# real-stanford/garmentnets

Measured on AMD Instinct MI355X. Metric: garments/s end-to-end predict (PointNet++ -> gridding -> UNet3D -> WNF decode -> marching cubes), higher is better.
Workload: dtype f32 (f16x2 convs, f16x2 decoder MLPs, fp32 accumulation)

## Files before the change

garmentnets_amd/csrc/upconv.hip:

```cpp
#include "split_conv.h"

struct UpArgs {
    const float *src;
    const float *a, *d;
    const uint4 *wp;
    const float *out_scale;
    const float *act_inv;
    float *partial;
    int C1, B, Dc, Hc, Wc, Cout;
    int tiles_y, tiles_x;
};

template <int NT, bool F16>
__global__ __launch_bounds__(512, 1) void upconv_partial_kernel(UpArgs p) {
    constexpr int TZC = NT == 1 ? 2 : 1, NF = 2 * TZC, HZ = TZC + 2, HVOX = HZ * 100;
    using HL = HaloLayout<2, HZ>;
    constexpr int NIT = (HVOX * 4 + 511) / 512;
    __shared__ __attribute__((aligned(16))) unsigned char smem[2 * HL::BYTES + 2 * 384 * 4];
    float *const adl = reinterpret_cast<float *>(smem + 2 * HL::BYTES);
    const int tid = threadIdx.x, lane = tid & 63, h = lane >> 5, r = lane & 31;
    const int cls = __builtin_amdgcn_readfirstlane(tid >> 6), pz = cls >> 2, py = (cls >> 1) & 1, px = cls & 1;
    const unsigned nblk = gridDim.x, xcd = blockIdx.x & 7u, jx = blockIdx.x >> 3, qx = nblk >> 3, rx = nblk & 7u;
    const unsigned logical = (xcd < rx ? xcd * (qx + 1) : rx * (qx + 1) + (xcd - rx) * qx) + jx;
    const int ncb = p.Cout / (32 * NT);
    int tile = (int)(logical / (unsigned)ncb);
    const int cb = (int)(logical % (unsigned)ncb);
    const int tiles_z = (p.Dc + TZC - 1) / TZC;
    const int tz = tile % tiles_z; tile /= tiles_z;
    const int tx = tile % p.tiles_x; tile /= p.tiles_x;
    const int ty = tile;
    const int z0 = tz * TZC, y0 = ty * 8, x0 = tx * 8;
    const int b = blockIdx.y;
    const int nslices = p.C1 / 16;
    const int nblocks = p.Cout / 32;

    f32x16 acc[NF][NT], tot[NF][NT];
#pragma unroll
    for (int f = 0; f < NF; ++f)
#pragma unroll
        for (int u = 0; u < NT; ++u)
#pragma unroll
            for (int q = 0; q < 16; ++q) { acc[f][u][q] = 0.f; tot[f][u][q] = 0.f; }
    for (int i = tid; i < p.C1; i += 512) { adl[i] = p.a[(int64_t)b * p.C1 + i]; adl[384 + i] = p.d[(int64_t)b * p.C1 + i]; }

    const int c4 = (tid & 3) * 4;
    float4 raw[NIT];
    unsigned inb = 0;
    auto issue_rows = [&](int sl) {
        inb = 0;
#pragma unroll
        for (int it = 0; it < NIT; ++it) {
            const int idx = tid + it * 512;
            const int hv = (idx < HVOX * 4 ? idx : HVOX * 4 - 1) >> 2;
            const int hx = hv % 10, hy = (hv / 10) % 10, hz = hv / 100;
            const int gz = z0 + hz - 1, gy = y0 + hy - 1, gx = x0 + hx - 1;
            const bool in = idx < HVOX * 4 && gz >= 0 && gz < p.Dc && gy >= 0 && gy < p.Hc && gx >= 0 && gx < p.Wc;
            raw[it] = make_float4(0.f, 0.f, 0.f, 0.f);
            if (in) {
                raw[it] = *reinterpret_cast<const float4 *>(p.src + ((((int64_t)b * p.Dc + gz) * p.Hc + gy) * p.Wc + gx) * p.C1 + sl * 16 + c4);
                inb |= 1u << it;
            }
        }
    };
    auto convert_row = [&](int it, int sl, int buf) {
        const int idx = tid + it * 512;
        if (idx < HVOX * 4) {
            const int hv = idx >> 2;
            const float4 av = *reinterpret_cast<const float4 *>(adl + sl * 16 + c4);
            const float4 dv = *reinterpret_cast<const float4 *>(adl + 384 + sl * 16 + c4);
            float v0 = 0.f, v1 = 0.f, v2 = 0.f, v3 = 0.f;
            if (inb & (1u << it)) {
                v0 = __fmaf_rn(raw[it].x, av.x, dv.x);
                v1 = __fmaf_rn(raw[it].y, av.y, dv.y);
                v2 = __fmaf_rn(raw[it].z, av.z, dv.z);
                v3 = __fmaf_rn(raw[it].w, av.w, dv.w);
            }
            uint2 pl[2];
            split4<2, F16>(v0, v1, v2, v3, pl);
            unsigned char *dst = smem + buf * HL::BYTES + HL::at(hv / 100, (hv / 10) % 10, hv % 10) + c4 * 2;
            *reinterpret_cast<uint2 *>(dst) = pl[0];
            *reinterpret_cast<uint2 *>(dst + 32) = pl[1];
        }
    };

    issue_rows(0);
    __syncthreads();
#pragma unroll
    for (int it = 0; it < NIT; ++it) convert_row(it, 0, 0);
    __syncthreads();

    const int64_t bstep = (int64_t)8 * nblocks * 2 * 64;
    const uint4 *bw = p.wp + ((int64_t)cls * nblocks + cb * NT) * 2 * 64 + lane;
    uint4 bf[NT][2], nbf[NT][2], nnbf[NT][2];
#pragma unroll
    for (int u = 0; u < NT; ++u) { nbf[u][0] = bw[(u * 2 + 0) * 64]; nbf[u][1] = bw[(u * 2 + 1) * 64]; }
    bw += bstep;
#pragma unroll
    for (int u = 0; u < NT; ++u) { nnbf[u][0] = bw[(u * 2 + 0) * 64]; nnbf[u][1] = bw[(u * 2 + 1) * 64]; }
    bw += bstep;
    const int abase = HL::at(pz, (r >> 3) + py, (r & 7) + px) + 16 * h;
    constexpr int AF1 = 4 * HL::ROWP, AFZ = 10 * HL::ROWP;
    const int nsteps = nslices * 8;
    int step = 0;
    uint4 af[NF][2], naf[NF][2];
#pragma unroll
    for (int f = 0; f < NF; ++f) {
        naf[f][0] = *reinterpret_cast<const uint4 *>(smem + abase + (f >> 1) * AFZ + (f & 1) * AF1);
        naf[f][1] = *reinterpret_cast<const uint4 *>(smem + abase + (f >> 1) * AFZ + (f & 1) * AF1 + 32);
    }
    for (int s = 0; s < nslices; ++s) {
        const unsigned char *const halo = smem + (s & 1) * HL::BYTES, *const halo_n = smem + ((s + 1) & 1) * HL::BYTES;
        const bool more = s + 1 < nslices;
        if (more) issue_rows(s + 1);
#pragma unroll
        for (int tap = 0; tap < 8; ++tap, ++step) {
#pragma unroll
            for (int u = 0; u < NT; ++u) { bf[u][0] = nbf[u][0]; bf[u][1] = nbf[u][1]; nbf[u][0] = nnbf[u][0]; nbf[u][1] = nnbf[u][1]; }
#pragma unroll
            for (int f = 0; f < NF; ++f) { af[f][0] = naf[f][0]; af[f][1] = naf[f][1]; }
            if (step + 2 < nsteps) {
#pragma unroll
                for (int u = 0; u < NT; ++u) { nnbf[u][0] = bw[(u * 2 + 0) * 64]; nnbf[u][1] = bw[(u * 2 + 1) * 64]; }
                bw += bstep;
            }
            if (tap < 7) {
                const int toff = HL::at((tap + 1) >> 2, ((tap + 1) >> 1) & 1, (tap + 1) & 1);
#pragma unroll
                for (int f = 0; f < NF; ++f) {
                    naf[f][0] = *reinterpret_cast<const uint4 *>(halo + abase + toff + (f >> 1) * AFZ + (f & 1) * AF1);
                    naf[f][1] = *reinterpret_cast<const uint4 *>(halo + abase + toff + (f >> 1) * AFZ + (f & 1) * AF1 + 32);
                }
            }
#define UP_PROD(IA, IB)                                                                                                        \
            _Pragma("unroll") for (int u = 0; u < NT; ++u)                                                                     \
                _Pragma("unroll") for (int f = 0; f < NF; ++f) acc[f][u] = mfma16<F16>(af[f][IA], bf[u][IB], acc[f][u]);
            UP_PROD(1, 0)
            if (more && tap >= 2 && tap < 2 + NIT) convert_row(tap - 2, s + 1, (s + 1) & 1);
            UP_PROD(0, 1) UP_PROD(0, 0)
#undef UP_PROD
        }
#pragma unroll
        for (int f = 0; f < NF; ++f)
#pragma unroll
            for (int u = 0; u < NT; ++u)
#pragma unroll
                for (int q = 0; q < 16; ++q) { tot[f][u][q] = __fadd_rn(tot[f][u][q], acc[f][u][q]); acc[f][u][q] = 0.f; }
        __syncthreads();
        if (more) {
#pragma unroll
            for (int f = 0; f < NF; ++f) {
                naf[f][0] = *reinterpret_cast<const uint4 *>(halo_n + abase + (f >> 1) * AFZ + (f & 1) * AF1);
                naf[f][1] = *reinterpret_cast<const uint4 *>(halo_n + abase + (f >> 1) * AFZ + (f & 1) * AF1 + 32);
            }
        }
    }
    const int64_t pc = (int64_t)8 * p.Cout;
#pragma unroll
    for (int f = 0; f < NF; ++f)
#pragma unroll
        for (int u = 0; u < NT; ++u) {
            const int t = f & 1, gz = z0 + (f >> 1);
            const int n = cls * p.Cout + (cb * NT + u) * 32 + r;
            const float osc = p.act_inv ? __fmul_rn(p.out_scale[n], p.act_inv[b]) : p.out_scale[n];
            if (z0 + TZC <= p.Dc && y0 + 8 <= p.Hc && x0 + 8 <= p.Wc) {
                float *ob = p.partial + ((((int64_t)b * p.Dc + gz) * p.Hc + (y0 + t * 4)) * p.Wc + (x0 + 4 * h)) * pc + n;
                const int64_t rs = (int64_t)p.Wc * pc;
#pragma unroll
                for (int q = 0; q < 16; ++q) ob[(q >> 2) * rs + (q & 3) * pc] = __fmul_rn(tot[f][u][q], osc);
                continue;
            }
#pragma unroll
            for (int q = 0; q < 16; ++q) {
                const int i = (q & 3) + 8 * (q >> 2) + 4 * h;
                const int gy = y0 + t * 4 + (i >> 3), gx = x0 + (i & 7);
                if (gz < p.Dc && gy < p.Hc && gx < p.Wc)
                    p.partial[((((int64_t)b * p.Dc + gz) * p.Hc + gy) * p.Wc + gx) * pc + n] = __fmul_rn(tot[f][u][q], osc);
            }
        }
}

extern "C" int gn_upconv_partial(const float *src1, int C1, const float *a, const float *d, const void *wp, int mode, const float *out_scale,
                                 const float *act_inv_scale, int B, int Dc, int Hc, int Wc, int Cout, float *partial, void *stream) {
    GN_REQUIRE(B >= 0 && Dc > 0 && Hc > 0 && Wc > 0 && C1 > 0 && Cout > 0, "gn_upconv_partial: bad sizes");
    GN_REQUIRE(mode == GN_SPLIT_BF16X2 || mode == GN_SPLIT_F16X2, "gn_upconv_partial: two-plane modes only (GN_SPLIT_BF16X2 / GN_SPLIT_F16X2)");
    GN_REQUIRE(C1 % 16 == 0 && C1 <= 384 && Cout % 32 == 0, "gn_upconv_partial: channels must be multiples of 16 (in, <= 384) / 32 (out)");
    if (B == 0) return GN_OK;
    GN_REQUIRE(src1 && a && d && wp && out_scale && partial, "gn_upconv_partial: null pointer");
    UpArgs p;
    p.src = src1; p.a = a; p.d = d; p.wp = (const uint4 *)wp; p.out_scale = out_scale; p.act_inv = act_inv_scale; p.partial = partial;
    p.C1 = C1; p.B = B; p.Dc = Dc; p.Hc = Hc; p.Wc = Wc; p.Cout = Cout;
    p.tiles_y = (int)gn_cdiv(Hc, 8); p.tiles_x = (int)gn_cdiv(Wc, 8);
    hipStream_t st = gn_stream(stream);
    const bool f16 = mode == GN_SPLIT_F16X2;
    if (Cout % 64 == 0) {
        const unsigned g = (unsigned)(gn_cdiv(Dc, 1) * p.tiles_y * p.tiles_x * (Cout / 64));
        if (f16) hipLaunchKernelGGL((upconv_partial_kernel<2, true>), dim3(g, B), dim3(512), 0, st, p);
        else hipLaunchKernelGGL((upconv_partial_kernel<2, false>), dim3(g, B), dim3(512), 0, st, p);
    } else {
        const unsigned g = (unsigned)(gn_cdiv(Dc, 2) * p.tiles_y * p.tiles_x * (Cout / 32));
        if (f16) hipLaunchKernelGGL((upconv_partial_kernel<1, true>), dim3(g, B), dim3(512), 0, st, p);
        else hipLaunchKernelGGL((upconv_partial_kernel<1, false>), dim3(g, B), dim3(512), 0, st, p);
    }
    GN_LAUNCH_CHECK("gn_upconv_partial");
    return GN_OK;
}
```

Measured before the change: 155.5.

## Make upconv kernel persistent with cross-tile prefetch of halo and weights

Converts the transposed-conv partial kernel into a persistent kernel launched with one block per CU (rounded to a multiple of 8). Each block loops over work items and overlaps the next tile's halo load, weight prefetch and per-sample affine table with the current tile's last slice. This is meant to hide the prologue and epilogue latency between tiles and to remove the cost of per-block launch and ramp-up. In exchange it adds complex control flow, a double-buffered affine table that uses more LDS, and possible load imbalance.

```diff
diff --git a/garmentnets_amd/csrc/upconv.hip b/garmentnets_amd/csrc/upconv.hip
--- a/garmentnets_amd/csrc/upconv.hip
+++ b/garmentnets_amd/csrc/upconv.hip
@@ -9,6 +9,7 @@
     float *partial;
     int C1, B, Dc, Hc, Wc, Cout;
     int tiles_y, tiles_x;
+    unsigned items_per_sample, n_items;
 };
 
 template <int NT, bool F16>
@@ -16,23 +17,27 @@
     constexpr int TZC = NT == 1 ? 2 : 1, NF = 2 * TZC, HZ = TZC + 2, HVOX = HZ * 100;
     using HL = HaloLayout<2, HZ>;
     constexpr int NIT = (HVOX * 4 + 511) / 512;
-    __shared__ __attribute__((aligned(16))) unsigned char smem[2 * HL::BYTES + 2 * 384 * 4];
+    __shared__ __attribute__((aligned(16))) unsigned char smem[2 * HL::BYTES + 2 * 2 * 384 * 4];
     float *const adl = reinterpret_cast<float *>(smem + 2 * HL::BYTES);
     const int tid = threadIdx.x, lane = tid & 63, h = lane >> 5, r = lane & 31;
     const int cls = __builtin_amdgcn_readfirstlane(tid >> 6), pz = cls >> 2, py = (cls >> 1) & 1, px = cls & 1;
-    const unsigned nblk = gridDim.x, xcd = blockIdx.x & 7u, jx = blockIdx.x >> 3, qx = nblk >> 3, rx = nblk & 7u;
-    const unsigned logical = (xcd < rx ? xcd * (qx + 1) : rx * (qx + 1) + (xcd - rx) * qx) + jx;
     const int ncb = p.Cout / (32 * NT);
-    int tile = (int)(logical / (unsigned)ncb);
-    const int cb = (int)(logical % (unsigned)ncb);
     const int tiles_z = (p.Dc + TZC - 1) / TZC;
-    const int tz = tile % tiles_z; tile /= tiles_z;
-    const int tx = tile % p.tiles_x; tile /= p.tiles_x;
-    const int ty = tile;
-    const int z0 = tz * TZC, y0 = ty * 8, x0 = tx * 8;
-    const int b = blockIdx.y;
     const int nslices = p.C1 / 16;
     const int nblocks = p.Cout / 32;
+    auto decode = [&](unsigned v, int &b_, int &cb_, int &z0_, int &y0_, int &x0_) {
+        const unsigned nblk = p.items_per_sample, bq = v / nblk, i = v - bq * nblk;
+        const unsigned xcd = i & 7u, jx = i >> 3, qx = nblk >> 3, rx = nblk & 7u;
+        const unsigned logical = (xcd < rx ? xcd * (qx + 1) : rx * (qx + 1) + (xcd - rx) * qx) + jx;
+        int tile = (int)(logical / (unsigned)ncb);
+        cb_ = (int)(logical % (unsigned)ncb);
+        const int tz = tile % tiles_z; tile /= tiles_z;
+        const int tx = tile % p.tiles_x; tile /= p.tiles_x;
+        b_ = (int)bq; z0_ = tz * TZC; y0_ = tile * 8; x0_ = tx * 8;
+    };
+    unsigned item = blockIdx.x;
+    int b, cb, z0, y0, x0;
+    decode(item, b, cb, z0, y0, x0);
 
     f32x16 acc[NF][NT], tot[NF][NT];
 #pragma unroll
@@ -41,33 +46,35 @@
         for (int u = 0; u < NT; ++u)
 #pragma unroll
             for (int q = 0; q < 16; ++q) { acc[f][u][q] = 0.f; tot[f][u][q] = 0.f; }
-    for (int i = tid; i < p.C1; i += 512) { adl[i] = p.a[(int64_t)b * p.C1 + i]; adl[384 + i] = p.d[(int64_t)b * p.C1 + i]; }
-
-    const int c4 = (tid & 3) * 4;
+
     float4 raw[NIT];
     unsigned inb = 0;
-    auto issue_rows = [&](int sl) {
+    auto issue_rows = [&](int b_, int z0_, int y0_, int x0_, int sl) {
         inb = 0;
+        int tl = threadIdx.x;
+        asm volatile("" : "+v"(tl));
 #pragma unroll
         for (int it = 0; it < NIT; ++it) {
-            const int idx = tid + it * 512;
+            const int idx = tl + it * 512;
             const int hv = (idx < HVOX * 4 ? idx : HVOX * 4 - 1) >> 2;
             const int hx = hv % 10, hy = (hv / 10) % 10, hz = hv / 100;
-            const int gz = z0 + hz - 1, gy = y0 + hy - 1, gx = x0 + hx - 1;
+            const int gz = z0_ + hz - 1, gy = y0_ + hy - 1, gx = x0_ + hx - 1;
             const bool in = idx < HVOX * 4 && gz >= 0 && gz < p.Dc && gy >= 0 && gy < p.Hc && gx >= 0 && gx < p.Wc;
             raw[it] = make_float4(0.f, 0.f, 0.f, 0.f);
             if (in) {
-                raw[it] = *reinterpret_cast<const float4 *>(p.src + ((((int64_t)b * p.Dc + gz) * p.Hc + gy) * p.Wc + gx) * p.C1 + sl * 16 + c4);
+                raw[it] = *reinterpret_cast<const float4 *>(p.src + ((((int64_t)b_ * p.Dc + gz) * p.Hc + gy) * p.Wc + gx) * p.C1 + sl * 16 + (tl & 3) * 4);
                 inb |= 1u << it;
             }
         }
     };
-    auto convert_row = [&](int it, int sl, int buf) {
-        const int idx = tid + it * 512;
+    auto convert_row = [&](int it, int sl, int buf, int tab) {
+        int tl = threadIdx.x;
+        asm volatile("" : "+v"(tl));
+        const int idx = tl + it * 512, c4 = (tl & 3) * 4;
         if (idx < HVOX * 4) {
             const int hv = idx >> 2;
-            const float4 av = *reinterpret_cast<const float4 *>(adl + sl * 16 + c4);
-            const float4 dv = *reinterpret_cast<const float4 *>(adl + 384 + sl * 16 + c4);
+            const float4 av = *reinterpret_cast<const float4 *>(adl + tab * 768 + sl * 16 + c4);
+            const float4 dv = *reinterpret_cast<const float4 *>(adl + tab * 768 + 384 + sl * 16 + c4);
             float v0 = 0.f, v1 = 0.f, v2 = 0.f, v3 = 0.f;
             if (inb & (1u << it)) {
                 v0 = __fmaf_rn(raw[it].x, av.x, dv.x);
@@ -83,100 +90,131 @@
         }
     };
 
-    issue_rows(0);
-    __syncthreads();
-#pragma unroll
-    for (int it = 0; it < NIT; ++it) convert_row(it, 0, 0);
-    __syncthreads();
-
     const int64_t bstep = (int64_t)8 * nblocks * 2 * 64;
-    const uint4 *bw = p.wp + ((int64_t)cls * nblocks + cb * NT) * 2 * 64 + lane;
+    auto bw_first = [&](int cb_) { return p.wp + ((int64_t)cls * nblocks + cb_ * NT) * 2 * 64 + lane; };
+    const uint4 *bw = nullptr;
     uint4 bf[NT][2], nbf[NT][2], nnbf[NT][2];
-#pragma unroll
-    for (int u = 0; u < NT; ++u) { nbf[u][0] = bw[(u * 2 + 0) * 64]; nbf[u][1] = bw[(u * 2 + 1) * 64]; }
-    bw += bstep;
-#pragma unroll
-    for (int u = 0; u < NT; ++u) { nnbf[u][0] = bw[(u * 2 + 0) * 64]; nnbf[u][1] = bw[(u * 2 + 1) * 64]; }
-    bw += bstep;
     const int abase = HL::at(pz, (r >> 3) + py, (r & 7) + px) + 16 * h;
     constexpr int AF1 = 4 * HL::ROWP, AFZ = 10 * HL::ROWP;
-    const int nsteps = nslices * 8;
-    int step = 0;
     uint4 af[NF][2], naf[NF][2];
-#pragma unroll
-    for (int f = 0; f < NF; ++f) {
-        naf[f][0] = *reinterpret_cast<const uint4 *>(smem + abase + (f >> 1) * AFZ + (f & 1) * AF1);
-        naf[f][1] = *reinterpret_cast<const uint4 *>(smem + abase + (f >> 1) * AFZ + (f & 1) * AF1 + 32);
+    const int64_t pc = (int64_t)8 * p.Cout;
+    bool fresh = true;
+    int buf = 0, tab = 0;
+    for (;;) {
+        const unsigned nitem = item + gridDim.x;
+        const bool more = nitem < p.n_items;
+        int bn = b, cbn = cb, z0n = z0, y0n = y0, x0n = x0;
+        if (more) decode(nitem, bn, cbn, z0n, y0n, x0n);
+        const bool cont = more && (bn == b || nslices >= 2);
+        const int tabn = bn == b ? tab : tab ^ 1;
+        if (fresh) {
+            __syncthreads();
+            for (int i = tid; i < p.C1; i += 512) { adl[tab * 768 + i] = p.a[(int64_t)b * p.C1 + i]; adl[tab * 768 + 384 + i] = p.d[(int64_t)b * p.C1 + i]; }
+            issue_rows(b, z0, y0, x0, 0);
+            __syncthreads();
+            buf = 0;
+#pragma unroll
+            for (int it = 0; it < NIT; ++it) convert_row(it, 0, 0, tab);
+            __syncthreads();
+            bw = bw_first(cb);
+#pragma unroll
+            for (int u = 0; u < NT; ++u) { nbf[u][0] = bw[(u * 2 + 0) * 64]; nbf[u][1] = bw[(u * 2 + 1) * 64]; }
+            bw += bstep;
+#pragma unroll
+            for (int u = 0; u < NT; ++u) { nnbf[u][0] = bw[(u * 2 + 0) * 64]; nnbf[u][1] = bw[(u * 2 + 1) * 64]; }
+            bw += bstep;
+#pragma unroll
+            for (int f = 0; f < NF; ++f) {
+                naf[f][0] = *reinterpret_cast<const uint4 *>(smem + abase + (f >> 1) * AFZ + (f & 1) * AF1);
+                naf[f][1] = *reinterpret_cast<const uint4 *>(smem + abase + (f >> 1) * AFZ + (f & 1) * AF1 + 32);
+            }
+            fresh = false;
+        }
+        for (int s = 0; s < nslices; ++s) {
+            const unsigned char *const halo = smem + buf * HL::BYTES, *const halo_n = smem + (buf ^ 1) * HL::BYTES;
+            const bool last = s + 1 == nslices;
+            const bool stage = !last || cont;
+            const int sls = last ? 0 : s + 1, tabs = last ? tabn : tab;
+            if (stage) issue_rows(last ? bn : b, last ? z0n : z0, last ? y0n : y0, last ? x0n : x0, sls);
+            const bool table = s == 0 && cont && bn != b && tid < p.C1;
+            float ta = 0.f, td = 0.f;
+#pragma unroll
+            for (int tap = 0; tap < 8; ++tap) {
+#pragma unroll
+                for (int u = 0; u < NT; ++u) { bf[u][0] = nbf[u][0]; bf[u][1] = nbf[u][1]; nbf[u][0] = nnbf[u][0]; nbf[u][1] = nnbf[u][1]; }
+#pragma unroll
+                for (int f = 0; f < NF; ++f) { af[f][0] = naf[f][0]; af[f][1] = naf[f][1]; }
+                if (last && tap == 6) bw = bw_first(cbn);
+                if (!last || tap < 6 || cont) {
+#pragma unroll
+                    for (int u = 0; u < NT; ++u) { nnbf[u][0] = bw[(u * 2 + 0) * 64]; nnbf[u][1] = bw[(u * 2 + 1) * 64]; }
+                    bw += bstep;
+                }
+                if (tap < 7) {
+                    const int toff = HL::at((tap + 1) >> 2, ((tap + 1) >> 1) & 1, (tap + 1) & 1);
+#pragma unroll
+                    for (int f = 0; f < NF; ++f) {
+                        naf[f][0] = *reinterpret_cast<const uint4 *>(halo + abase + toff + (f >> 1) * AFZ + (f & 1) * AF1);
+                        naf[f][1] = *reinterpret_cast<const uint4 *>(halo + abase + toff + (f >> 1) * AFZ + (f & 1) * AF1 + 32);
+                    }
+                }
+                if (tap == 6 && table) { ta = p.a[(int64_t)bn * p.C1 + tid]; td = p.d[(int64_t)bn * p.C1 + tid]; }
+#define UP_PROD(IA, IB)                                                                                                        \
+                _Pragma("unroll") for (int u = 0; u < NT; ++u)                                                                 \
+                    _Pragma("unroll") for (int f = 0; f < NF; ++f) acc[f][u] = mfma16<F16>(af[f][IA], bf[u][IB], acc[f][u]);
+                UP_PROD(1, 0)
+                if (stage && tap >= 2 && tap < 2 + NIT) convert_row(tap - 2, sls, buf ^ 1, tabs);
+                UP_PROD(0, 1) UP_PROD(0, 0)
+#undef UP_PROD
+            }
+            if (table) { adl[(tab ^ 1) * 768 + tid] = ta; adl[(tab ^ 1) * 768 + 384 + tid] = td; }
+#pragma unroll
+            for (int f = 0; f < NF; ++f)
+#pragma unroll
+                for (int u = 0; u < NT; ++u)
+#pragma unroll
+                    for (int q = 0; q < 16; ++q) { tot[f][u][q] = __fadd_rn(tot[f][u][q], acc[f][u][q]); acc[f][u][q] = 0.f; }
+            __syncthreads();
+            if (stage) {
+#pragma unroll
+                for (int f = 0; f < NF; ++f) {
+                    naf[f][0] = *reinterpret_cast<const uint4 *>(halo_n + abase + (f >> 1) * AFZ + (f & 1) * AF1);
+                    naf[f][1] = *reinterpret_cast<const uint4 *>(halo_n + abase + (f >> 1) * AFZ + (f & 1) * AF1 + 32);
+                }
+            }
+            buf ^= 1;
+        }
+        int le = threadIdx.x;
+        asm volatile("" : "+v"(le));
+        const int re = le & 31, he = (le >> 5) & 1;
+#pragma unroll
+        for (int f = 0; f < NF; ++f)
+#pragma unroll
+            for (int u = 0; u < NT; ++u) {
+                const int t = f & 1, gz = z0 + (f >> 1);
+                const int n = cls * p.Cout + (cb * NT + u) * 32 + re;
+                const float osc = p.act_inv ? __fmul_rn(p.out_scale[n], p.act_inv[b]) : p.out_scale[n];
+                if (z0 + TZC <= p.Dc && y0 + 8 <= p.Hc && x0 + 8 <= p.Wc) {
+                    float *ob = p.partial + ((((int64_t)b * p.Dc + gz) * p.Hc + (y0 + t * 4)) * p.Wc + (x0 + 4 * he)) * pc + n;
+                    const int64_t rs = (int64_t)p.Wc * pc;
+#pragma unroll
+                    for (int q = 0; q < 16; ++q) { ob[(q >> 2) * rs + (q & 3) * pc] = __fmul_rn(tot[f][u][q], osc); tot[f][u][q] = 0.f; }
+                    continue;
+                }
+#pragma unroll
+                for (int q = 0; q < 16; ++q) {
+                    const int i = (q & 3) + 8 * (q >> 2) + 4 * he;
+                    const int gy = y0 + t * 4 + (i >> 3), gx = x0 + (i & 7);
+                    if (gz < p.Dc && gy < p.Hc && gx < p.Wc)
+                        p.partial[((((int64_t)b * p.Dc + gz) * p.Hc + gy) * p.Wc + gx) * pc + n] = __fmul_rn(tot[f][u][q], osc);
+                    tot[f][u][q] = 0.f;
+                }
+            }
+        if (!more) break;
+        fresh = !cont;
+        tab = tabn;
+        item = nitem; b = bn; cb = cbn; z0 = z0n; y0 = y0n; x0 = x0n;
     }
-    for (int s = 0; s < nslices; ++s) {
-        const unsigned char *const halo = smem + (s & 1) * HL::BYTES, *const halo_n = smem + ((s + 1) & 1) * HL::BYTES;
-        const bool more = s + 1 < nslices;
-        if (more) issue_rows(s + 1);
-#pragma unroll
-        for (int tap = 0; tap < 8; ++tap, ++step) {
-#pragma unroll
-            for (int u = 0; u < NT; ++u) { bf[u][0] = nbf[u][0]; bf[u][1] = nbf[u][1]; nbf[u][0] = nnbf[u][0]; nbf[u][1] = nnbf[u][1]; }
-#pragma unroll
-            for (int f = 0; f < NF; ++f) { af[f][0] = naf[f][0]; af[f][1] = naf[f][1]; }
-            if (step + 2 < nsteps) {
-#pragma unroll
-                for (int u = 0; u < NT; ++u) { nnbf[u][0] = bw[(u * 2 + 0) * 64]; nnbf[u][1] = bw[(u * 2 + 1) * 64]; }
-                bw += bstep;
-            }
-            if (tap < 7) {
-                const int toff = HL::at((tap + 1) >> 2, ((tap + 1) >> 1) & 1, (tap + 1) & 1);
-#pragma unroll
-                for (int f = 0; f < NF; ++f) {
-                    naf[f][0] = *reinterpret_cast<const uint4 *>(halo + abase + toff + (f >> 1) * AFZ + (f & 1) * AF1);
-                    naf[f][1] = *reinterpret_cast<const uint4 *>(halo + abase + toff + (f >> 1) * AFZ + (f & 1) * AF1 + 32);
-                }
-            }
-#define UP_PROD(IA, IB)                                                                                                        \
-            _Pragma("unroll") for (int u = 0; u < NT; ++u)                                                                     \
-                _Pragma("unroll") for (int f = 0; f < NF; ++f) acc[f][u] = mfma16<F16>(af[f][IA], bf[u][IB], acc[f][u]);
-            UP_PROD(1, 0)
-            if (more && tap >= 2 && tap < 2 + NIT) convert_row(tap - 2, s + 1, (s + 1) & 1);
-            UP_PROD(0, 1) UP_PROD(0, 0)
-#undef UP_PROD
-        }
-#pragma unroll
-        for (int f = 0; f < NF; ++f)
-#pragma unroll
-            for (int u = 0; u < NT; ++u)
-#pragma unroll
-                for (int q = 0; q < 16; ++q) { tot[f][u][q] = __fadd_rn(tot[f][u][q], acc[f][u][q]); acc[f][u][q] = 0.f; }
-        __syncthreads();
-        if (more) {
-#pragma unroll
-            for (int f = 0; f < NF; ++f) {
-                naf[f][0] = *reinterpret_cast<const uint4 *>(halo_n + abase + (f >> 1) * AFZ + (f & 1) * AF1);
-                naf[f][1] = *reinterpret_cast<const uint4 *>(halo_n + abase + (f >> 1) * AFZ + (f & 1) * AF1 + 32);
-            }
-        }
-    }
-    const int64_t pc = (int64_t)8 * p.Cout;
-#pragma unroll
-    for (int f = 0; f < NF; ++f)
-#pragma unroll
-        for (int u = 0; u < NT; ++u) {
-            const int t = f & 1, gz = z0 + (f >> 1);
-            const int n = cls * p.Cout + (cb * NT + u) * 32 + r;
-            const float osc = p.act_inv ? __fmul_rn(p.out_scale[n], p.act_inv[b]) : p.out_scale[n];
-            if (z0 + TZC <= p.Dc && y0 + 8 <= p.Hc && x0 + 8 <= p.Wc) {
-                float *ob = p.partial + ((((int64_t)b * p.Dc + gz) * p.Hc + (y0 + t * 4)) * p.Wc + (x0 + 4 * h)) * pc + n;
-                const int64_t rs = (int64_t)p.Wc * pc;
-#pragma unroll
-                for (int q = 0; q < 16; ++q) ob[(q >> 2) * rs + (q & 3) * pc] = __fmul_rn(tot[f][u][q], osc);
-                continue;
-            }
-#pragma unroll
-            for (int q = 0; q < 16; ++q) {
-                const int i = (q & 3) + 8 * (q >> 2) + 4 * h;
-                const int gy = y0 + t * 4 + (i >> 3), gx = x0 + (i & 7);
-                if (gz < p.Dc && gy < p.Hc && gx < p.Wc)
-                    p.partial[((((int64_t)b * p.Dc + gz) * p.Hc + gy) * p.Wc + gx) * pc + n] = __fmul_rn(tot[f][u][q], osc);
-            }
-        }
 }
 
 extern "C" int gn_upconv_partial(const float *src1, int C1, const float *a, const float *d, const void *wp, int mode, const float *out_scale,
@@ -192,14 +230,23 @@
     p.tiles_y = (int)gn_cdiv(Hc, 8); p.tiles_x = (int)gn_cdiv(Wc, 8);
     hipStream_t st = gn_stream(stream);
     const bool f16 = mode == GN_SPLIT_F16X2;
-    if (Cout % 64 == 0) {
-        const unsigned g = (unsigned)(gn_cdiv(Dc, 1) * p.tiles_y * p.tiles_x * (Cout / 64));
-        if (f16) hipLaunchKernelGGL((upconv_partial_kernel<2, true>), dim3(g, B), dim3(512), 0, st, p);
-        else hipLaunchKernelGGL((upconv_partial_kernel<2, false>), dim3(g, B), dim3(512), 0, st, p);
+    const int nt = Cout % 64 == 0 ? 2 : 1;
+    const int64_t per_sample = gn_cdiv(Dc, nt == 2 ? 1 : 2) * p.tiles_y * p.tiles_x * (Cout / (32 * nt));
+    GN_REQUIRE(per_sample * B < (int64_t)1 << 31, "gn_upconv_partial: too many tiles");
+    p.items_per_sample = (unsigned)per_sample; p.n_items = (unsigned)(per_sample * B);
+    static const int cus = [] {
+        int dev = 0, n = 256;
+        hipDeviceProp_t pr;
+        if (hipGetDevice(&dev) == hipSuccess && hipGetDeviceProperties(&pr, dev) == hipSuccess && pr.multiProcessorCount >= 8) n = pr.multiProcessorCount & ~7;
+        return n;
+    }();
+    const unsigned g = p.n_items < (unsigned)cus ? p.n_items : (unsigned)cus;
+    if (nt == 2) {
+        if (f16) hipLaunchKernelGGL((upconv_partial_kernel<2, true>), dim3(g), dim3(512), 0, st, p);
+        else hipLaunchKernelGGL((upconv_partial_kernel<2, false>), dim3(g), dim3(512), 0, st, p);
     } else {
-        const unsigned g = (unsigned)(gn_cdiv(Dc, 2) * p.tiles_y * p.tiles_x * (Cout / 32));
-        if (f16) hipLaunchKernelGGL((upconv_partial_kernel<1, true>), dim3(g, B), dim3(512), 0, st, p);
-        else hipLaunchKernelGGL((upconv_partial_kernel<1, false>), dim3(g, B), dim3(512), 0, st, p);
+        if (f16) hipLaunchKernelGGL((upconv_partial_kernel<1, true>), dim3(g), dim3(512), 0, st, p);
+        else hipLaunchKernelGGL((upconv_partial_kernel<1, false>), dim3(g), dim3(512), 0, st, p);
     }
     GN_LAUNCH_CHECK("gn_upconv_partial");
     return GN_OK;
```

Result: no change. 155.4 (median of 2 runs) (-0.0%).
